# cloneofsimo/paint-with-words-sd

Hardware: NVIDIA H100
Metric: unet_steps_per_sec_512sq_cfg (higher is better)
Workload: dtype f16

## Files before the change

paint_with_words_sd_b200/csrc/attn_tc.cuh:

```cuda
#pragma once
#include "mma_sm90.cuh"
#include "pww_common.cuh"
#include "xattn_core.cuh"

namespace pww {
namespace fa {

constexpr int kThreads = core::kThreads;
constexpr int kBM = core::kBM;
constexpr int kBN = 64;

template <int D>
struct Cfg {
  using T_ = core::Tile<D>;
  static constexpr uint32_t KVBYTES = kBN * T_::LD * 2;
  static constexpr uint32_t OFF_KV = T_::QBYTES;
  static constexpr uint32_t SMEM = T_::QBYTES + 2 * 2 * KVBYTES;
  static_assert(SMEM <= 232448, "shared memory budget");
};

template <typename E>
struct Params {
  const E* q;
  const E* k;
  const E* v;
  E* out;
  int B, H, N;
  int64_t bs, rs;
  int64_t o_bs, o_rs;
  float scale;
};

template <int D, typename E>
constexpr int kMinBlocks = (D == 80 && std::is_same_v<E, __nv_bfloat16>) ? 1 : 0;

template <int D, typename E>
__global__ void __launch_bounds__(kThreads, kMinBlocks<D, E>) attn_fwd_kernel(const Params<E> p) {
  using C = core::Tile<D>;
  using CF = Cfg<D>;
  extern __shared__ __align__(128) unsigned char smem[];
  const uint32_t smem0 = ptx::smem_u32(smem);
  const int warp = threadIdx.x >> 5, lane = threadIdx.x & 31;
  const int qtiles = (p.N + kBM - 1) / kBM;
  const int bh = blockIdx.x / qtiles, qt = blockIdx.x - bh * qtiles;
  const int b = bh / p.H, h = bh - b * p.H;
  const int row_base = qt * kBM;
  const E* qb = p.q + (int64_t)b * p.bs + h * D;
  const E* kb = p.k + (int64_t)b * p.bs + h * D;
  const E* vb = p.v + (int64_t)b * p.bs + h * D;
  const int ntiles = (p.N + kBN - 1) / kBN;
  auto issue_kv = [&](int j) {
    const uint32_t st = smem0 + CF::OFF_KV + (j & 1) * 2 * CF::KVBYTES;
    const int rows = p.N - j * kBN < kBN ? p.N - j * kBN : kBN;
    core::load_rows<D>(st, kb + (int64_t)j * kBN * p.rs, p.rs, kBN, rows);
    core::load_rows<D>(st + CF::KVBYTES, vb + (int64_t)j * kBN * p.rs, p.rs, kBN, rows);
    ptx::cp_async_commit();
  };
  {
    const int rows = p.N - row_base < kBM ? p.N - row_base : kBM;
    core::load_rows<D>(smem0, qb + (int64_t)row_base * p.rs, p.rs, kBM, rows);
  }
  issue_kv(0);
  uint32_t qa[C::KS][4];
  float o[C::NT][4], m0, m1, l0, l1;
  core::warp_online_begin<D>(o, m0, m1, l0, l1);
  const float sl2 = p.scale * 1.4426950408889634f;
  const uint32_t qs = smem0 + (uint32_t)(warp * 16 * C::LD) * 2u;
#pragma unroll 1
  for (int jt = 0; jt < ntiles; ++jt) {
    if (jt + 1 < ntiles) {
      issue_kv(jt + 1);
      ptx::cp_async_wait<1>();
    } else {
      ptx::cp_async_wait<0>();
    }
    __syncthreads();
    if (jt == 0) {
#pragma unroll
      for (int kk = 0; kk < C::KS; ++kk)
        ptx::ldsm_x4(qs + (uint32_t)((lane & 15) * C::LD + kk * 16 + (lane >> 4) * 8) * 2u, qa[kk][0], qa[kk][1], qa[kk][2], qa[kk][3]);
    }
    const uint32_t ks = smem0 + CF::OFF_KV + (jt & 1) * 2 * CF::KVBYTES, vs = ks + CF::KVBYTES;
    float s[kBN / 8][4];
#pragma unroll
    for (int j = 0; j < kBN / 8; ++j) s[j][0] = s[j][1] = s[j][2] = s[j][3] = 0.f;
#pragma unroll
    for (int kk = 0; kk < C::KS; ++kk) {
#pragma unroll
      for (int jp = 0; jp < kBN / 16; ++jp) {
        const int t = 16 * jp + (lane & 7) + ((lane >> 4) << 3), d = kk * 16 + ((lane >> 3) & 1) * 8;
        uint32_t b0, b1, b2, b3;
        ptx::ldsm_x4(ks + (uint32_t)(t * C::LD + d) * 2u, b0, b1, b2, b3);
        ptx::mma16816<E>(s[2 * jp], qa[kk], b0, b1);
        ptx::mma16816<E>(s[2 * jp + 1], qa[kk], b2, b3);
      }
    }
    core::warp_online_chunk<D, E>(s, p.N - jt * kBN, sl2, vs, lane, o, m0, m1, l0, l1);
    __syncthreads();
  }
  core::warp_online_end<D>(o, l0, l1);
  core::warp_store<D>(o, smem + warp * 16 * C::LD * 2, lane, p.out + (int64_t)b * p.o_bs + h * D, p.o_rs,
                      row_base + warp * 16, p.N);
}

template <int D, typename E>
cudaError_t launch(const void* q, const void* k, const void* v, void* out, int B, int H, int N, int64_t bs, int64_t rs,
                   int64_t o_bs, int64_t o_rs, float scale, cudaStream_t s) {
  using CF = Cfg<D>;
  Params<E> p;
  p.q = (const E*)q; p.k = (const E*)k; p.v = (const E*)v; p.out = (E*)out;
  p.B = B; p.H = H; p.N = N; p.bs = bs; p.rs = rs; p.o_bs = o_bs; p.o_rs = o_rs; p.scale = scale;
  const cudaError_t e = allow_dynamic_smem<attn_fwd_kernel<D, E>>(CF::SMEM);
  if (e != cudaSuccess) return e;
  const long long grid = (long long)B * H * ((N + kBM - 1) / kBM);
  if (grid > 0x7fffffffLL) return cudaErrorInvalidConfiguration;
  attn_fwd_kernel<D, E><<<(unsigned)grid, kThreads, CF::SMEM, s>>>(p);
  return cudaGetLastError();
}

}
}
```

paint_with_words_sd_b200/csrc/mma_sm90.cuh:

```cuda
#pragma once
#include <cuda_runtime.h>
#include <stdint.h>

#include <type_traits>

#include "pww_common.cuh"

namespace pww {
namespace ptx {

__device__ __forceinline__ uint32_t smem_u32(const void* p) { return (uint32_t)__cvta_generic_to_shared(p); }

__device__ __forceinline__ void cp_async16(uint32_t dst, const void* src, uint32_t src_bytes) {
  asm volatile("cp.async.cg.shared.global [%0], [%1], 16, %2;" ::"r"(dst), "l"(src), "r"(src_bytes) : "memory");
}
__device__ __forceinline__ void cp_async_commit() { asm volatile("cp.async.commit_group;" ::: "memory"); }
template <int N>
__device__ __forceinline__ void cp_async_wait() { asm volatile("cp.async.wait_group %0;" ::"n"(N) : "memory"); }

__device__ __forceinline__ void ldsm_x4(uint32_t addr, uint32_t& r0, uint32_t& r1, uint32_t& r2, uint32_t& r3) {
  asm volatile("ldmatrix.sync.aligned.m8n8.x4.shared.b16 {%0, %1, %2, %3}, [%4];"
               : "=r"(r0), "=r"(r1), "=r"(r2), "=r"(r3) : "r"(addr));
}
__device__ __forceinline__ void ldsm_x4_t(uint32_t addr, uint32_t& r0, uint32_t& r1, uint32_t& r2, uint32_t& r3) {
  asm volatile("ldmatrix.sync.aligned.m8n8.x4.trans.shared.b16 {%0, %1, %2, %3}, [%4];"
               : "=r"(r0), "=r"(r1), "=r"(r2), "=r"(r3) : "r"(addr));
}
__device__ __forceinline__ void ldsm_x2_t(uint32_t addr, uint32_t& r0, uint32_t& r1) {
  asm volatile("ldmatrix.sync.aligned.m8n8.x2.trans.shared.b16 {%0, %1}, [%2];" : "=r"(r0), "=r"(r1) : "r"(addr));
}

template <typename E>
__device__ __forceinline__ void mma16816(float* c, const uint32_t* a, uint32_t b0, uint32_t b1) {
  static_assert(std::is_same_v<E, __half> || std::is_same_v<E, __nv_bfloat16>, "fp16 or bf16 operands");
  if constexpr (std::is_same_v<E, __half>) {
    asm volatile(
        "mma.sync.aligned.m16n8k16.row.col.f32.f16.f16.f32 {%0, %1, %2, %3}, {%4, %5, %6, %7}, {%8, %9}, "
        "{%0, %1, %2, %3};"
        : "+f"(c[0]), "+f"(c[1]), "+f"(c[2]), "+f"(c[3])
        : "r"(a[0]), "r"(a[1]), "r"(a[2]), "r"(a[3]), "r"(b0), "r"(b1));
  } else {
    asm volatile(
        "mma.sync.aligned.m16n8k16.row.col.f32.bf16.bf16.f32 {%0, %1, %2, %3}, {%4, %5, %6, %7}, {%8, %9}, "
        "{%0, %1, %2, %3};"
        : "+f"(c[0]), "+f"(c[1]), "+f"(c[2]), "+f"(c[3])
        : "r"(a[0]), "r"(a[1]), "r"(a[2]), "r"(a[3]), "r"(b0), "r"(b1));
  }
}

__device__ __forceinline__ float ex2(float x) {
  float y;
  asm("ex2.approx.ftz.f32 %0, %1;" : "=f"(y) : "f"(x));
  return y;
}
template <typename E>
__device__ __forceinline__ uint32_t pack2(float lo, float hi) {
  const typename Elem<E>::E2 h = Elem<E>::from_float2(lo, hi);
  return *reinterpret_cast<const uint32_t*>(&h);
}
template <typename E>
__device__ __forceinline__ float2 unpack2(uint32_t v) {
  return Elem<E>::to_float2(*reinterpret_cast<const typename Elem<E>::E2*>(&v));
}
__device__ __forceinline__ unsigned long long ld_acquire_gpu_u64(const unsigned long long* p) {
  unsigned long long v;
  asm volatile("ld.acquire.gpu.global.u64 %0, [%1];" : "=l"(v) : "l"(p) : "memory");
  return v;
}

}
}
```

paint_with_words_sd_b200/csrc/xattn_core.cuh:

```cuda
#pragma once
#include "mma_sm90.cuh"
#include "pww_common.cuh"

namespace pww {
namespace core {

constexpr int kBM = 128;
constexpr int kTP = 80;
constexpr int kWarps = 8;
constexpr int kThreads = kWarps * 32;

template <int D>
struct Tile {
  static_assert(D == 40 || D == 64 || D == 80 || D == 160, "head dims of SD1.5 (40 / 80 / 160) and SD2.x (64)");
  static constexpr int DP = (D + 15) / 16 * 16;
  static constexpr int LD = DP + 8;
  static constexpr int KS = DP / 16;
  static constexpr int NT = D / 8;
  static constexpr uint32_t QBYTES = kBM * LD * 2;
  static constexpr uint32_t KBYTES = kTP * LD * 2;
};

template <int D, typename E>
__device__ __forceinline__ void load_rows(uint32_t dst, const E* src, int64_t rs, int nrows, int valid) {
  using C = Tile<D>;
  constexpr int CH = C::DP / 8, DCH = D / 8;
  for (int idx = threadIdx.x; idx < nrows * CH; idx += blockDim.x) {
    const int r = idx / CH, c = idx - r * CH;
    const bool ok = r < valid && c < DCH;
    ptx::cp_async16(dst + (uint32_t)(r * C::LD + c * 8) * 2u, ok ? (const void*)(src + (int64_t)r * rs + c * 8) : (const void*)src,
                    ok ? 16u : 0u);
  }
}

template <int D, typename E>
__device__ __forceinline__ void warp_qk(uint32_t qs, uint32_t ks, int lane, float (&s)[10][4]) {
  using C = Tile<D>;
#pragma unroll
  for (int j = 0; j < 10; ++j) s[j][0] = s[j][1] = s[j][2] = s[j][3] = 0.f;
#pragma unroll
  for (int kk = 0; kk < C::KS; ++kk) {
    uint32_t a[4];
    ptx::ldsm_x4(qs + (uint32_t)((lane & 15) * C::LD + kk * 16 + (lane >> 4) * 8) * 2u, a[0], a[1], a[2], a[3]);
#pragma unroll
    for (int jp = 0; jp < 5; ++jp) {
      const int t = 16 * jp + (lane & 7) + ((lane >> 4) << 3), d = kk * 16 + ((lane >> 3) & 1) * 8;
      uint32_t b0, b1, b2, b3;
      ptx::ldsm_x4(ks + (uint32_t)(t * C::LD + d) * 2u, b0, b1, b2, b3);
      ptx::mma16816<E>(s[2 * jp], a, b0, b1);
      ptx::mma16816<E>(s[2 * jp + 1], a, b2, b3);
    }
  }
}

__device__ __forceinline__ int tok(int j, int e, int lane) { return 8 * j + 2 * (lane & 3) + (e & 1); }

template <int D, typename E>
__device__ __forceinline__ void warp_store(const float (&o)[Tile<D>::NT][4], unsigned char* stage, int lane, E* out,
                                           int64_t o_rs, int row0, int N) {
  using C = Tile<D>;
  __syncwarp();
  const int g = lane >> 2, q = lane & 3;
#pragma unroll
  for (int j = 0; j < C::NT; ++j) {
    *reinterpret_cast<uint32_t*>(stage + (g * C::LD + 8 * j + 2 * q) * 2) = ptx::pack2<E>(o[j][0], o[j][1]);
    *reinterpret_cast<uint32_t*>(stage + ((g + 8) * C::LD + 8 * j + 2 * q) * 2) = ptx::pack2<E>(o[j][2], o[j][3]);
  }
  __syncwarp();
  for (int idx = lane; idx < 16 * C::NT; idx += 32) {
    const int r = idx / C::NT, c = idx - r * C::NT;
    if (row0 + r < N)
      *reinterpret_cast<uint4*>(out + (int64_t)(row0 + r) * o_rs + c * 8) =
          *reinterpret_cast<const uint4*>(stage + (r * C::LD + c * 8) * 2);
  }
  __syncwarp();
}

constexpr int kChunk = 77;
constexpr int kMaxChunks = 3;
__host__ __device__ __forceinline__ constexpr int chunks_of(int T) { return T <= kTP ? 1 : T / kChunk; }
__host__ __device__ __forceinline__ constexpr bool supported_keys(int T) {
  return T <= kTP || T == 2 * kChunk || T == kMaxChunks * kChunk;
}
template <int KC>
__host__ __device__ __forceinline__ constexpr int chunk_keys(int T) { return KC == 1 ? T : kChunk; }

template <int D, int KC, typename E>
__device__ __forceinline__ void load_operands(uint32_t st, const XattnParams<E>& p, int b, int h, int tile, bool with_v) {
  using C = Tile<D>;
  const int rows = p.N - tile * kBM;
  load_rows<D>(st, p.q + (int64_t)b * p.q_bs + (int64_t)tile * kBM * p.q_rs + h * D, p.q_rs, kBM, rows < kBM ? rows : kBM);
  const int kv = chunk_keys<KC>(p.T);
#pragma unroll 1
  for (int c = 0; c < KC; ++c) {
    const int64_t off = (int64_t)b * p.k_bs + (int64_t)c * kChunk * p.k_rs + h * D;
    load_rows<D>(st + C::QBYTES + c * C::KBYTES, p.k + off, p.k_rs, kTP, kv);
    if (with_v) load_rows<D>(st + C::QBYTES + (KC + c) * C::KBYTES, p.v + off, p.k_rs, kTP, kv);
  }
}

template <int D>
__device__ __forceinline__ void warp_online_begin(float (&o)[Tile<D>::NT][4], float& m0, float& m1, float& l0, float& l1) {
#pragma unroll
  for (int j = 0; j < Tile<D>::NT; ++j) o[j][0] = o[j][1] = o[j][2] = o[j][3] = 0.f;
  m0 = m1 = -INFINITY;
  l0 = l1 = 0.f;
}

struct NoPHook {
  template <int NK>
  __device__ __forceinline__ void operator()(const uint32_t (&)[NK][4], float, float) const {}
};

template <int D, typename E, int NJ, typename Hook = NoPHook>
__device__ __forceinline__ void warp_online_chunk(float (&s)[NJ][4], int kv, float sl2, uint32_t vs, int lane,
                                                  float (&o)[Tile<D>::NT][4], float& m0, float& m1, float& l0, float& l1,
                                                  const Hook& hook = Hook{}) {
  static_assert(NJ % 2 == 0, "P V takes two n-tiles of P per k-step");
  using C = Tile<D>;
  float t0 = -INFINITY, t1 = -INFINITY;
#pragma unroll
  for (int j = 0; j < NJ; ++j)
#pragma unroll
    for (int e = 0; e < 4; ++e) {
      if (tok(j, e, lane) >= kv) s[j][e] = -INFINITY;
      if (e < 2) t0 = fmaxf(t0, s[j][e]); else t1 = fmaxf(t1, s[j][e]);
    }
  t0 = fmaxf(t0, __shfl_xor_sync(0xffffffffu, t0, 1));
  t0 = fmaxf(t0, __shfl_xor_sync(0xffffffffu, t0, 2));
  t1 = fmaxf(t1, __shfl_xor_sync(0xffffffffu, t1, 1));
  t1 = fmaxf(t1, __shfl_xor_sync(0xffffffffu, t1, 2));
  const float mn0 = fmaxf(m0, t0), mn1 = fmaxf(m1, t1);
  const float a0 = ptx::ex2((m0 - mn0) * sl2), a1 = ptx::ex2((m1 - mn1) * sl2);
  m0 = mn0; m1 = mn1;
  const float n0 = -mn0 * sl2, n1 = -mn1 * sl2;
  uint32_t pa[NJ / 2][4];
  float r0 = 0.f, r1 = 0.f;
#pragma unroll
  for (int j = 0; j < NJ; ++j) {
    const uint32_t p01 = ptx::pack2<E>(ptx::ex2(fmaf(s[j][0], sl2, n0)), ptx::ex2(fmaf(s[j][1], sl2, n0)));
    const uint32_t p23 = ptx::pack2<E>(ptx::ex2(fmaf(s[j][2], sl2, n1)), ptx::ex2(fmaf(s[j][3], sl2, n1)));
    const float2 f01 = ptx::unpack2<E>(p01), f23 = ptx::unpack2<E>(p23);
    r0 += f01.x + f01.y;
    r1 += f23.x + f23.y;
    pa[j >> 1][(j & 1) * 2] = p01;
    pa[j >> 1][(j & 1) * 2 + 1] = p23;
  }
  l0 = l0 * a0 + r0;
  l1 = l1 * a1 + r1;
#pragma unroll
  for (int j = 0; j < C::NT; ++j) {
    o[j][0] *= a0; o[j][1] *= a0; o[j][2] *= a1; o[j][3] *= a1;
  }
#pragma unroll
  for (int kk = 0; kk < NJ / 2; ++kk) {
    const int t = 16 * kk + (lane & 7) + ((lane >> 3) & 1) * 8;
#pragma unroll
    for (int jp = 0; jp < C::NT / 2; ++jp) {
      uint32_t b0, b1, b2, b3;
      ptx::ldsm_x4_t(vs + (uint32_t)(t * C::LD + 16 * jp + (lane >> 4) * 8) * 2u, b0, b1, b2, b3);
      ptx::mma16816<E>(o[2 * jp], pa[kk], b0, b1);
      ptx::mma16816<E>(o[2 * jp + 1], pa[kk], b2, b3);
    }
    if constexpr (C::NT & 1) {
      uint32_t b0, b1;
      ptx::ldsm_x2_t(vs + (uint32_t)(t * C::LD + 8 * (C::NT - 1)) * 2u, b0, b1);
      ptx::mma16816<E>(o[C::NT - 1], pa[kk], b0, b1);
    }
  }
  hook(pa, a0, a1);
}

template <int D>
__device__ __forceinline__ void warp_online_end(float (&o)[Tile<D>::NT][4], float l0, float l1) {
  l0 += __shfl_xor_sync(0xffffffffu, l0, 1);
  l0 += __shfl_xor_sync(0xffffffffu, l0, 2);
  l1 += __shfl_xor_sync(0xffffffffu, l1, 1);
  l1 += __shfl_xor_sync(0xffffffffu, l1, 2);
  const float i0 = 1.f / l0, i1 = 1.f / l1;
#pragma unroll
  for (int j = 0; j < Tile<D>::NT; ++j) {
    o[j][0] *= i0; o[j][1] *= i0; o[j][2] *= i1; o[j][3] *= i1;
  }
}

constexpr int kRegions = 16;

template <typename E, int NK>
__device__ __forceinline__ void warp_region_chunk(const uint32_t (&pa)[NK][4], float a0, float a1, const int8_t* rt,
                                                  int lane, float (&rm)[2][4]) {
#pragma unroll
  for (int j = 0; j < 2; ++j) {
    rm[j][0] *= a0; rm[j][1] *= a0; rm[j][2] *= a1; rm[j][3] *= a1;
  }
  const int r = lane >> 2;
#pragma unroll
  for (int kk = 0; kk < NK; ++kk) {
    const int t = 16 * kk + 2 * (lane & 3);
    const int i0 = __ldg(rt + t), i1 = __ldg(rt + t + 1), i2 = __ldg(rt + t + 8), i3 = __ldg(rt + t + 9);
#pragma unroll
    for (int j = 0; j < 2; ++j) {
      const int slot = r + 8 * j;
      const uint32_t b0 = ptx::pack2<E>(i0 == slot ? 1.f : 0.f, i1 == slot ? 1.f : 0.f);
      const uint32_t b1 = ptx::pack2<E>(i2 == slot ? 1.f : 0.f, i3 == slot ? 1.f : 0.f);
      ptx::mma16816<E>(rm[j], pa[kk], b0, b1);
    }
  }
}

__device__ __forceinline__ void warp_region_add(const float (&rm)[2][4], float l0, float l1, float* acc, int row0, int N,
                                                int lane) {
  l0 += __shfl_xor_sync(0xffffffffu, l0, 1);
  l0 += __shfl_xor_sync(0xffffffffu, l0, 2);
  l1 += __shfl_xor_sync(0xffffffffu, l1, 1);
  l1 += __shfl_xor_sync(0xffffffffu, l1, 2);
  const float inv[2] = {1.f / l0, 1.f / l1};
  const int g = lane >> 2, q = lane & 3;
#pragma unroll
  for (int hf = 0; hf < 2; ++hf) {
    const int row = row0 + g + 8 * hf;
    if (row >= N) continue;
    float* a = acc + (int64_t)row * kRegions + 2 * q;
#pragma unroll
    for (int j = 0; j < 2; ++j) {
      a[8 * j] += rm[j][2 * hf] * inv[hf];
      a[8 * j + 1] += rm[j][2 * hf + 1] * inv[hf];
    }
  }
}

template <typename E>
__device__ __forceinline__ void warp_stat(const float (&s)[10][4], int T, int rows_left, int lane, bool is_max, float& vmax,
                                          float& sum, float& sumsq) {
  const int g = lane >> 2;
#pragma unroll
  for (int j = 0; j < 10; ++j)
#pragma unroll
    for (int e = 0; e < 4; ++e) {
      const bool ok = tok(j, e, lane) < T && (g + (e >> 1) * 8) < rows_left;
      if (is_max) {
        if (ok) vmax = fmaxf(vmax, s[j][e]);
      } else if (ok) {
        const float h = round_to<E>(s[j][e]);
        sum += h;
        sumsq = fmaf(h, h, sumsq);
      }
    }
}

__device__ __forceinline__ void warp_reduce_stat(double& m, double& a, double& q) {
#pragma unroll
  for (int o = 16; o > 0; o >>= 1) {
    m = fmax(m, __shfl_xor_sync(0xffffffffu, m, o));
    a += __shfl_xor_sync(0xffffffffu, a, o);
    q += __shfl_xor_sync(0xffffffffu, q, o);
  }
}

template <typename E>
__device__ __forceinline__ float stat_value(const XattnParams<E>& p, bool is_max, double m, double a, double q) {
  const double cnt = (double)p.H * (double)p.N * (double)p.T;
  double r;
  if (is_max) {
    r = m;
  } else {
    const double var = (q - a * a / cnt) / (cnt - 1.0);
    r = sqrt(var > 0.0 ? var : 0.0);
  }
  return round_to<E>((float)r);
}

}
}
```

Measured before the change: 160.0.

## Port self-attention kernel from mma.sync to Hopper wgmma with swizzled smem

Replaces the warp-level mma.sync and ldmatrix attention inner loop with warpgroup wgmma: QK^T runs from smem descriptors over 128B-swizzled tiles, and PV uses register-A wgmma. The softmax row sum is folded into the PV MMA by appending a constant-one column to V, and the unmasked tiles take a no-mask path. It also uses a larger key tile for head dim 40 and a two-stage prefetch issued after the barrier. This is meant to cut ldmatrix and issue overhead and raise tensor core throughput, at the cost of extra padding columns, fp16 rounding of the row sum, and a fragile descriptor and swizzle setup.

```diff
diff --git a/paint_with_words_sd_b200/csrc/attn_tc.cuh b/paint_with_words_sd_b200/csrc/attn_tc.cuh
--- a/paint_with_words_sd_b200/csrc/attn_tc.cuh
+++ b/paint_with_words_sd_b200/csrc/attn_tc.cuh
@@ -8,16 +8,6 @@
 
 constexpr int kThreads = core::kThreads;
 constexpr int kBM = core::kBM;
-constexpr int kBN = 64;
-
-template <int D>
-struct Cfg {
-  using T_ = core::Tile<D>;
-  static constexpr uint32_t KVBYTES = kBN * T_::LD * 2;
-  static constexpr uint32_t OFF_KV = T_::QBYTES;
-  static constexpr uint32_t SMEM = T_::QBYTES + 2 * 2 * KVBYTES;
-  static_assert(SMEM <= 232448, "shared memory budget");
-};
 
 template <typename E>
 struct Params {
@@ -31,15 +21,55 @@
   float scale;
 };
 
-template <int D, typename E>
-constexpr int kMinBlocks = (D == 80 && std::is_same_v<E, __nv_bfloat16>) ? 1 : 0;
+template <int D>
+struct WgCfg {
+  static constexpr int BN = D == 40 ? 128 : 64;
+  static constexpr int DP = core::Tile<D>::DP;
+  static constexpr int KS = DP / 16;
+  static constexpr int NO = D / 8 + 1;
+  static constexpr int KA = (DP / 8 + 7) / 8, VA = (NO + 7) / 8;
+  static constexpr uint32_t QBYTES = KA * kBM * 128, KBYTES = KA * BN * 128, VBYTES = VA * BN * 128;
+  static constexpr uint32_t STAGE = KBYTES + VBYTES;
+  static constexpr uint32_t SMEM = 1024 + QBYTES + 2 * STAGE;
+  static constexpr int MIN_BLOCKS = D <= 80 ? 2 : 1;
+  static_assert(SMEM * MIN_BLOCKS <= 227 * 1024, "shared memory budget");
+  static_assert(kBM * core::Tile<D>::LD * 2 <= QBYTES + 2 * STAGE, "the output staging fits the operand buffers");
+};
+
+template <int ROWS>
+__device__ __forceinline__ uint32_t sw128_off(int r, int c) {
+  return (uint32_t)((c >> 3) * ROWS * 128 + r * 128 + (((c & 7) ^ (r & 7)) << 4));
+}
+
+template <int ROWS, int D, typename E>
+__device__ __forceinline__ void copy_rows(uint32_t dst, const E* src, int64_t rs, int valid) {
+  constexpr int TPR = kThreads / ROWS, DC = D / 8;
+  const int r = threadIdx.x / TPR, c0 = threadIdx.x % TPR;
+  const bool ok = r < valid;
+  const E* row = src + (int64_t)r * rs;
+#pragma unroll
+  for (int i = 0; i < (DC + TPR - 1) / TPR; ++i) {
+    const int c = c0 + TPR * i;
+    if (DC % TPR == 0 || c < DC)
+      ptx::cp_async16(dst + sw128_off<ROWS>(r, c), ok ? (const void*)(row + c * 8) : (const void*)src, ok ? 16u : 0u);
+  }
+}
+
+template <int ROWS, int D>
+__device__ __forceinline__ void put_constant_chunk(unsigned char* dst, uint32_t first_word) {
+  constexpr int TPR = kThreads / ROWS;
+  if (threadIdx.x % TPR == 0)
+    *reinterpret_cast<uint4*>(dst + sw128_off<ROWS>(threadIdx.x / TPR, D / 8)) = make_uint4(first_word, 0u, 0u, 0u);
+}
 
 template <int D, typename E>
-__global__ void __launch_bounds__(kThreads, kMinBlocks<D, E>) attn_fwd_kernel(const Params<E> p) {
+__global__ void __launch_bounds__(kThreads, WgCfg<D>::MIN_BLOCKS) attn_fwd_kernel(const Params<E> p) {
   using C = core::Tile<D>;
-  using CF = Cfg<D>;
+  using W = WgCfg<D>;
+  constexpr int BN = W::BN;
   extern __shared__ __align__(128) unsigned char smem[];
-  const uint32_t smem0 = ptx::smem_u32(smem);
+  const uint32_t raw = ptx::smem_u32(smem), base = (raw + 1023u) & ~1023u;
+  unsigned char* const gbase = smem + (base - raw);
   const int warp = threadIdx.x >> 5, lane = threadIdx.x & 31;
   const int qtiles = (p.N + kBM - 1) / kBM;
   const int bh = blockIdx.x / qtiles, qt = blockIdx.x - bh * qtiles;
@@ -48,73 +78,88 @@
   const E* qb = p.q + (int64_t)b * p.bs + h * D;
   const E* kb = p.k + (int64_t)b * p.bs + h * D;
   const E* vb = p.v + (int64_t)b * p.bs + h * D;
-  const int ntiles = (p.N + kBN - 1) / kBN;
+  const int ntiles = (p.N + BN - 1) / BN;
   auto issue_kv = [&](int j) {
-    const uint32_t st = smem0 + CF::OFF_KV + (j & 1) * 2 * CF::KVBYTES;
-    const int rows = p.N - j * kBN < kBN ? p.N - j * kBN : kBN;
-    core::load_rows<D>(st, kb + (int64_t)j * kBN * p.rs, p.rs, kBN, rows);
-    core::load_rows<D>(st + CF::KVBYTES, vb + (int64_t)j * kBN * p.rs, p.rs, kBN, rows);
+    const uint32_t st = base + W::QBYTES + (j & 1) * W::STAGE;
+    const int rows = p.N - j * BN < BN ? p.N - j * BN : BN;
+    copy_rows<BN, D>(st, kb + (int64_t)j * BN * p.rs, p.rs, rows);
+    copy_rows<BN, D>(st + W::KBYTES, vb + (int64_t)j * BN * p.rs, p.rs, rows);
     ptx::cp_async_commit();
   };
   {
     const int rows = p.N - row_base < kBM ? p.N - row_base : kBM;
-    core::load_rows<D>(smem0, qb + (int64_t)row_base * p.rs, p.rs, kBM, rows);
+    copy_rows<kBM, D>(base, qb + (int64_t)row_base * p.rs, p.rs, rows);
   }
   issue_kv(0);
-  uint32_t qa[C::KS][4];
-  float o[C::NT][4], m0, m1, l0, l1;
-  core::warp_online_begin<D>(o, m0, m1, l0, l1);
+  if (ntiles > 1) issue_kv(1);
+  {
+    const uint32_t one = ptx::pack2<E>(1.f, 0.f);
+    if constexpr (W::DP > D) put_constant_chunk<kBM, D>(gbase, 0u);
+#pragma unroll
+    for (int st = 0; st < 2; ++st) {
+      unsigned char* const s = gbase + W::QBYTES + st * W::STAGE;
+      if constexpr (W::DP > D) put_constant_chunk<BN, D>(s, 0u);
+      put_constant_chunk<BN, D>(s + W::KBYTES, one);
+    }
+  }
+  float o[W::NO][4], m0 = -INFINITY, m1 = -INFINITY;
+#pragma unroll
+  for (int j = 0; j < W::NO; ++j) o[j][0] = o[j][1] = o[j][2] = o[j][3] = 0.f;
+  auto& od = reinterpret_cast<float(&)[C::NT][4]>(o);
+  float l0 = 0.f, l1 = 0.f;
   const float sl2 = p.scale * 1.4426950408889634f;
-  const uint32_t qs = smem0 + (uint32_t)(warp * 16 * C::LD) * 2u;
+  const uint32_t qs = base + (uint32_t)(warp >> 2) * 64 * 128;
 #pragma unroll 1
   for (int jt = 0; jt < ntiles; ++jt) {
-    if (jt + 1 < ntiles) {
-      issue_kv(jt + 1);
-      ptx::cp_async_wait<1>();
-    } else {
-      ptx::cp_async_wait<0>();
-    }
+    if (jt + 1 < ntiles) ptx::cp_async_wait<1>(); else ptx::cp_async_wait<0>();
+    ptx::fence_proxy_async();
     __syncthreads();
-    if (jt == 0) {
+    const uint32_t ks = base + W::QBYTES + (jt & 1) * W::STAGE, vs = ks + W::KBYTES;
+    float s[BN / 8][4];
+    ptx::wgmma_fence();
 #pragma unroll
-      for (int kk = 0; kk < C::KS; ++kk)
-        ptx::ldsm_x4(qs + (uint32_t)((lane & 15) * C::LD + kk * 16 + (lane >> 4) * 8) * 2u, qa[kk][0], qa[kk][1], qa[kk][2], qa[kk][3]);
-    }
-    const uint32_t ks = smem0 + CF::OFF_KV + (jt & 1) * 2 * CF::KVBYTES, vs = ks + CF::KVBYTES;
-    float s[kBN / 8][4];
+    for (int kk = 0; kk < W::KS; ++kk)
+      ptx::wgmma_ss<BN, E>(s, ptx::sw128_desc(qs + (kk >> 2) * kBM * 128 + (kk & 3) * 32, 16, 1024),
+                           ptx::sw128_desc(ks + (kk >> 2) * BN * 128 + (kk & 3) * 32, 16, 1024), kk > 0);
+    ptx::wgmma_commit();
+    ptx::wgmma_wait<0>();
+    ptx::reg_fence(s);
+    uint32_t pa[BN / 16][4];
+    float a0, a1;
+    const int kv = p.N - jt * BN;
+    if (kv >= BN)
+      core::warp_online_softmax<D, E, BN / 8, false, false>(s, kv, sl2, lane, od, m0, m1, l0, l1, pa, a0, a1);
+    else
+      core::warp_online_softmax<D, E, BN / 8, true, false>(s, kv, sl2, lane, od, m0, m1, l0, l1, pa, a0, a1);
+    o[W::NO - 1][0] *= a0; o[W::NO - 1][1] *= a0; o[W::NO - 1][2] *= a1; o[W::NO - 1][3] *= a1;
+    ptx::reg_fence(o);
+    ptx::wgmma_fence();
 #pragma unroll
-    for (int j = 0; j < kBN / 8; ++j) s[j][0] = s[j][1] = s[j][2] = s[j][3] = 0.f;
-#pragma unroll
-    for (int kk = 0; kk < C::KS; ++kk) {
-#pragma unroll
-      for (int jp = 0; jp < kBN / 16; ++jp) {
-        const int t = 16 * jp + (lane & 7) + ((lane >> 4) << 3), d = kk * 16 + ((lane >> 3) & 1) * 8;
-        uint32_t b0, b1, b2, b3;
-        ptx::ldsm_x4(ks + (uint32_t)(t * C::LD + d) * 2u, b0, b1, b2, b3);
-        ptx::mma16816<E>(s[2 * jp], qa[kk], b0, b1);
-        ptx::mma16816<E>(s[2 * jp + 1], qa[kk], b2, b3);
-      }
-    }
-    core::warp_online_chunk<D, E>(s, p.N - jt * kBN, sl2, vs, lane, o, m0, m1, l0, l1);
+    for (int kk = 0; kk < BN / 16; ++kk)
+      ptx::wgmma_rs<8 * W::NO, E>(o, pa[kk], ptx::sw128_desc(vs + kk * 16 * 128, BN * 128, 1024));
+    ptx::wgmma_commit();
+    ptx::wgmma_wait<0>();
+    ptx::reg_fence(o);
     __syncthreads();
+    if (jt + 2 < ntiles) issue_kv(jt + 2);
   }
-  core::warp_online_end<D>(o, l0, l1);
-  core::warp_store<D>(o, smem + warp * 16 * C::LD * 2, lane, p.out + (int64_t)b * p.o_bs + h * D, p.o_rs,
+  core::warp_online_end<D>(od, o[W::NO - 1][0] + o[W::NO - 1][1], o[W::NO - 1][2] + o[W::NO - 1][3]);
+  core::warp_store<D>(od, gbase + warp * 16 * C::LD * 2, lane, p.out + (int64_t)b * p.o_bs + h * D, p.o_rs,
                       row_base + warp * 16, p.N);
 }
 
 template <int D, typename E>
 cudaError_t launch(const void* q, const void* k, const void* v, void* out, int B, int H, int N, int64_t bs, int64_t rs,
                    int64_t o_bs, int64_t o_rs, float scale, cudaStream_t s) {
-  using CF = Cfg<D>;
+  using W = WgCfg<D>;
   Params<E> p;
   p.q = (const E*)q; p.k = (const E*)k; p.v = (const E*)v; p.out = (E*)out;
   p.B = B; p.H = H; p.N = N; p.bs = bs; p.rs = rs; p.o_bs = o_bs; p.o_rs = o_rs; p.scale = scale;
-  const cudaError_t e = allow_dynamic_smem<attn_fwd_kernel<D, E>>(CF::SMEM);
+  const cudaError_t e = allow_dynamic_smem<attn_fwd_kernel<D, E>>(W::SMEM);
   if (e != cudaSuccess) return e;
   const long long grid = (long long)B * H * ((N + kBM - 1) / kBM);
   if (grid > 0x7fffffffLL) return cudaErrorInvalidConfiguration;
-  attn_fwd_kernel<D, E><<<(unsigned)grid, kThreads, CF::SMEM, s>>>(p);
+  attn_fwd_kernel<D, E><<<(unsigned)grid, kThreads, W::SMEM, s>>>(p);
   return cudaGetLastError();
 }
 
diff --git a/paint_with_words_sd_b200/csrc/mma_sm90.cuh b/paint_with_words_sd_b200/csrc/mma_sm90.cuh
--- a/paint_with_words_sd_b200/csrc/mma_sm90.cuh
+++ b/paint_with_words_sd_b200/csrc/mma_sm90.cuh
@@ -48,6 +48,144 @@
   }
 }
 
+__device__ __forceinline__ uint64_t sw128_desc(uint32_t addr, uint32_t lbo, uint32_t sbo) {
+  return (uint64_t)((addr & 0x3FFFFu) >> 4) | ((uint64_t)((lbo >> 4) & 0x3FFFu) << 16) |
+         ((uint64_t)((sbo >> 4) & 0x3FFFu) << 32) | (1ull << 62);
+}
+__device__ __forceinline__ void fence_proxy_async() { asm volatile("fence.proxy.async.shared::cta;" ::: "memory"); }
+__device__ __forceinline__ void wgmma_fence() { asm volatile("wgmma.fence.sync.aligned;" ::: "memory"); }
+__device__ __forceinline__ void wgmma_commit() { asm volatile("wgmma.commit_group.sync.aligned;" ::: "memory"); }
+template <int N>
+__device__ __forceinline__ void wgmma_wait() { asm volatile("wgmma.wait_group.sync.aligned %0;" ::"n"(N) : "memory"); }
+template <int R>
+__device__ __forceinline__ void reg_fence(float (&x)[R][4]) {
+#pragma unroll
+  for (int i = 0; i < R; ++i) asm volatile("" : "+f"(x[i][0]), "+f"(x[i][1]), "+f"(x[i][2]), "+f"(x[i][3])::"memory");
+}
+
+#define PWW_WG_REGS_48 "{%0, %1, %2, %3, %4, %5, %6, %7, %8, %9, %10, %11, %12, %13, %14, %15" \
+  ", %16, %17, %18, %19, %20, %21, %22, %23}"
+#define PWW_WG_OUT_48(d) "+f"(d[0][0]), "+f"(d[0][1]), "+f"(d[0][2]), "+f"(d[0][3]), "+f"(d[1][0]), "+f"(d[1][1]), \
+  "+f"(d[1][2]), "+f"(d[1][3]), "+f"(d[2][0]), "+f"(d[2][1]), "+f"(d[2][2]), "+f"(d[2][3]), "+f"(d[3][0]), \
+  "+f"(d[3][1]), "+f"(d[3][2]), "+f"(d[3][3]), "+f"(d[4][0]), "+f"(d[4][1]), "+f"(d[4][2]), "+f"(d[4][3]), \
+  "+f"(d[5][0]), "+f"(d[5][1]), "+f"(d[5][2]), "+f"(d[5][3])
+#define PWW_WG_REGS_64 "{%0, %1, %2, %3, %4, %5, %6, %7, %8, %9, %10, %11, %12, %13, %14, %15" \
+  ", %16, %17, %18, %19, %20, %21, %22, %23, %24, %25, %26, %27, %28, %29, %30, %31}"
+#define PWW_WG_OUT_64(d) "+f"(d[0][0]), "+f"(d[0][1]), "+f"(d[0][2]), "+f"(d[0][3]), "+f"(d[1][0]), "+f"(d[1][1]), \
+  "+f"(d[1][2]), "+f"(d[1][3]), "+f"(d[2][0]), "+f"(d[2][1]), "+f"(d[2][2]), "+f"(d[2][3]), "+f"(d[3][0]), \
+  "+f"(d[3][1]), "+f"(d[3][2]), "+f"(d[3][3]), "+f"(d[4][0]), "+f"(d[4][1]), "+f"(d[4][2]), "+f"(d[4][3]), \
+  "+f"(d[5][0]), "+f"(d[5][1]), "+f"(d[5][2]), "+f"(d[5][3]), "+f"(d[6][0]), "+f"(d[6][1]), "+f"(d[6][2]), \
+  "+f"(d[6][3]), "+f"(d[7][0]), "+f"(d[7][1]), "+f"(d[7][2]), "+f"(d[7][3])
+#define PWW_WG_REGS_72 "{%0, %1, %2, %3, %4, %5, %6, %7, %8, %9, %10, %11, %12, %13, %14, %15" \
+  ", %16, %17, %18, %19, %20, %21, %22, %23, %24, %25, %26, %27, %28, %29, %30, %31" \
+  ", %32, %33, %34, %35}"
+#define PWW_WG_OUT_72(d) "+f"(d[0][0]), "+f"(d[0][1]), "+f"(d[0][2]), "+f"(d[0][3]), "+f"(d[1][0]), "+f"(d[1][1]), \
+  "+f"(d[1][2]), "+f"(d[1][3]), "+f"(d[2][0]), "+f"(d[2][1]), "+f"(d[2][2]), "+f"(d[2][3]), "+f"(d[3][0]), \
+  "+f"(d[3][1]), "+f"(d[3][2]), "+f"(d[3][3]), "+f"(d[4][0]), "+f"(d[4][1]), "+f"(d[4][2]), "+f"(d[4][3]), \
+  "+f"(d[5][0]), "+f"(d[5][1]), "+f"(d[5][2]), "+f"(d[5][3]), "+f"(d[6][0]), "+f"(d[6][1]), "+f"(d[6][2]), \
+  "+f"(d[6][3]), "+f"(d[7][0]), "+f"(d[7][1]), "+f"(d[7][2]), "+f"(d[7][3]), "+f"(d[8][0]), "+f"(d[8][1]), \
+  "+f"(d[8][2]), "+f"(d[8][3])
+#define PWW_WG_REGS_88 "{%0, %1, %2, %3, %4, %5, %6, %7, %8, %9, %10, %11, %12, %13, %14, %15" \
+  ", %16, %17, %18, %19, %20, %21, %22, %23, %24, %25, %26, %27, %28, %29, %30, %31" \
+  ", %32, %33, %34, %35, %36, %37, %38, %39, %40, %41, %42, %43}"
+#define PWW_WG_OUT_88(d) "+f"(d[0][0]), "+f"(d[0][1]), "+f"(d[0][2]), "+f"(d[0][3]), "+f"(d[1][0]), "+f"(d[1][1]), \
+  "+f"(d[1][2]), "+f"(d[1][3]), "+f"(d[2][0]), "+f"(d[2][1]), "+f"(d[2][2]), "+f"(d[2][3]), "+f"(d[3][0]), \
+  "+f"(d[3][1]), "+f"(d[3][2]), "+f"(d[3][3]), "+f"(d[4][0]), "+f"(d[4][1]), "+f"(d[4][2]), "+f"(d[4][3]), \
+  "+f"(d[5][0]), "+f"(d[5][1]), "+f"(d[5][2]), "+f"(d[5][3]), "+f"(d[6][0]), "+f"(d[6][1]), "+f"(d[6][2]), \
+  "+f"(d[6][3]), "+f"(d[7][0]), "+f"(d[7][1]), "+f"(d[7][2]), "+f"(d[7][3]), "+f"(d[8][0]), "+f"(d[8][1]), \
+  "+f"(d[8][2]), "+f"(d[8][3]), "+f"(d[9][0]), "+f"(d[9][1]), "+f"(d[9][2]), "+f"(d[9][3]), "+f"(d[10][0]), \
+  "+f"(d[10][1]), "+f"(d[10][2]), "+f"(d[10][3])
+#define PWW_WG_REGS_128 "{%0, %1, %2, %3, %4, %5, %6, %7, %8, %9, %10, %11, %12, %13, %14, %15" \
+  ", %16, %17, %18, %19, %20, %21, %22, %23, %24, %25, %26, %27, %28, %29, %30, %31" \
+  ", %32, %33, %34, %35, %36, %37, %38, %39, %40, %41, %42, %43, %44, %45, %46, %47" \
+  ", %48, %49, %50, %51, %52, %53, %54, %55, %56, %57, %58, %59, %60, %61, %62, %63}"
+#define PWW_WG_OUT_128(d) "+f"(d[0][0]), "+f"(d[0][1]), "+f"(d[0][2]), "+f"(d[0][3]), "+f"(d[1][0]), "+f"(d[1][1]), \
+  "+f"(d[1][2]), "+f"(d[1][3]), "+f"(d[2][0]), "+f"(d[2][1]), "+f"(d[2][2]), "+f"(d[2][3]), "+f"(d[3][0]), \
+  "+f"(d[3][1]), "+f"(d[3][2]), "+f"(d[3][3]), "+f"(d[4][0]), "+f"(d[4][1]), "+f"(d[4][2]), "+f"(d[4][3]), \
+  "+f"(d[5][0]), "+f"(d[5][1]), "+f"(d[5][2]), "+f"(d[5][3]), "+f"(d[6][0]), "+f"(d[6][1]), "+f"(d[6][2]), \
+  "+f"(d[6][3]), "+f"(d[7][0]), "+f"(d[7][1]), "+f"(d[7][2]), "+f"(d[7][3]), "+f"(d[8][0]), "+f"(d[8][1]), \
+  "+f"(d[8][2]), "+f"(d[8][3]), "+f"(d[9][0]), "+f"(d[9][1]), "+f"(d[9][2]), "+f"(d[9][3]), "+f"(d[10][0]), \
+  "+f"(d[10][1]), "+f"(d[10][2]), "+f"(d[10][3]), "+f"(d[11][0]), "+f"(d[11][1]), "+f"(d[11][2]), "+f"(d[11][3]), \
+  "+f"(d[12][0]), "+f"(d[12][1]), "+f"(d[12][2]), "+f"(d[12][3]), "+f"(d[13][0]), "+f"(d[13][1]), "+f"(d[13][2]), \
+  "+f"(d[13][3]), "+f"(d[14][0]), "+f"(d[14][1]), "+f"(d[14][2]), "+f"(d[14][3]), "+f"(d[15][0]), "+f"(d[15][1]), \
+  "+f"(d[15][2]), "+f"(d[15][3])
+#define PWW_WG_REGS_168 "{%0, %1, %2, %3, %4, %5, %6, %7, %8, %9, %10, %11, %12, %13, %14, %15" \
+  ", %16, %17, %18, %19, %20, %21, %22, %23, %24, %25, %26, %27, %28, %29, %30, %31" \
+  ", %32, %33, %34, %35, %36, %37, %38, %39, %40, %41, %42, %43, %44, %45, %46, %47" \
+  ", %48, %49, %50, %51, %52, %53, %54, %55, %56, %57, %58, %59, %60, %61, %62, %63" \
+  ", %64, %65, %66, %67, %68, %69, %70, %71, %72, %73, %74, %75, %76, %77, %78, %79" \
+  ", %80, %81, %82, %83}"
+#define PWW_WG_OUT_168(d) "+f"(d[0][0]), "+f"(d[0][1]), "+f"(d[0][2]), "+f"(d[0][3]), "+f"(d[1][0]), "+f"(d[1][1]), \
+  "+f"(d[1][2]), "+f"(d[1][3]), "+f"(d[2][0]), "+f"(d[2][1]), "+f"(d[2][2]), "+f"(d[2][3]), "+f"(d[3][0]), \
+  "+f"(d[3][1]), "+f"(d[3][2]), "+f"(d[3][3]), "+f"(d[4][0]), "+f"(d[4][1]), "+f"(d[4][2]), "+f"(d[4][3]), \
+  "+f"(d[5][0]), "+f"(d[5][1]), "+f"(d[5][2]), "+f"(d[5][3]), "+f"(d[6][0]), "+f"(d[6][1]), "+f"(d[6][2]), \
+  "+f"(d[6][3]), "+f"(d[7][0]), "+f"(d[7][1]), "+f"(d[7][2]), "+f"(d[7][3]), "+f"(d[8][0]), "+f"(d[8][1]), \
+  "+f"(d[8][2]), "+f"(d[8][3]), "+f"(d[9][0]), "+f"(d[9][1]), "+f"(d[9][2]), "+f"(d[9][3]), "+f"(d[10][0]), \
+  "+f"(d[10][1]), "+f"(d[10][2]), "+f"(d[10][3]), "+f"(d[11][0]), "+f"(d[11][1]), "+f"(d[11][2]), "+f"(d[11][3]), \
+  "+f"(d[12][0]), "+f"(d[12][1]), "+f"(d[12][2]), "+f"(d[12][3]), "+f"(d[13][0]), "+f"(d[13][1]), "+f"(d[13][2]), \
+  "+f"(d[13][3]), "+f"(d[14][0]), "+f"(d[14][1]), "+f"(d[14][2]), "+f"(d[14][3]), "+f"(d[15][0]), "+f"(d[15][1]), \
+  "+f"(d[15][2]), "+f"(d[15][3]), "+f"(d[16][0]), "+f"(d[16][1]), "+f"(d[16][2]), "+f"(d[16][3]), "+f"(d[17][0]), \
+  "+f"(d[17][1]), "+f"(d[17][2]), "+f"(d[17][3]), "+f"(d[18][0]), "+f"(d[18][1]), "+f"(d[18][2]), "+f"(d[18][3]), \
+  "+f"(d[19][0]), "+f"(d[19][1]), "+f"(d[19][2]), "+f"(d[19][3]), "+f"(d[20][0]), "+f"(d[20][1]), "+f"(d[20][2]), \
+  "+f"(d[20][3])
+#define PWW_WGMMA_SS_64(T, d, da, db, sc) \
+  asm volatile("{\n.reg .pred p;\nsetp.ne.b32 p, %34, 0;\n" \
+               "wgmma.mma_async.sync.aligned.m64n64k16.f32." T "." T " " PWW_WG_REGS_64 \
+               ", %32, %33, p, 1, 1, 0, 0;\n}\n" \
+               : PWW_WG_OUT_64(d) : "l"(da), "l"(db), "r"(sc))
+#define PWW_WGMMA_SS_128(T, d, da, db, sc) \
+  asm volatile("{\n.reg .pred p;\nsetp.ne.b32 p, %66, 0;\n" \
+               "wgmma.mma_async.sync.aligned.m64n128k16.f32." T "." T " " PWW_WG_REGS_128 \
+               ", %64, %65, p, 1, 1, 0, 0;\n}\n" \
+               : PWW_WG_OUT_128(d) : "l"(da), "l"(db), "r"(sc))
+#define PWW_WGMMA_RS_48(T, d, a, db) \
+  asm volatile("{\n.reg .pred p;\nsetp.ne.b32 p, %29, 0;\n" \
+               "wgmma.mma_async.sync.aligned.m64n48k16.f32." T "." T " " PWW_WG_REGS_48 \
+               ", {%24, %25, %26, %27}, %28, p, 1, 1, 1;\n}\n" \
+               : PWW_WG_OUT_48(d) : "r"(a[0]), "r"(a[1]), "r"(a[2]), "r"(a[3]), "l"(db), "r"(1))
+#define PWW_WGMMA_RS_72(T, d, a, db) \
+  asm volatile("{\n.reg .pred p;\nsetp.ne.b32 p, %41, 0;\n" \
+               "wgmma.mma_async.sync.aligned.m64n72k16.f32." T "." T " " PWW_WG_REGS_72 \
+               ", {%36, %37, %38, %39}, %40, p, 1, 1, 1;\n}\n" \
+               : PWW_WG_OUT_72(d) : "r"(a[0]), "r"(a[1]), "r"(a[2]), "r"(a[3]), "l"(db), "r"(1))
+#define PWW_WGMMA_RS_88(T, d, a, db) \
+  asm volatile("{\n.reg .pred p;\nsetp.ne.b32 p, %49, 0;\n" \
+               "wgmma.mma_async.sync.aligned.m64n88k16.f32." T "." T " " PWW_WG_REGS_88 \
+               ", {%44, %45, %46, %47}, %48, p, 1, 1, 1;\n}\n" \
+               : PWW_WG_OUT_88(d) : "r"(a[0]), "r"(a[1]), "r"(a[2]), "r"(a[3]), "l"(db), "r"(1))
+#define PWW_WGMMA_RS_168(T, d, a, db) \
+  asm volatile("{\n.reg .pred p;\nsetp.ne.b32 p, %89, 0;\n" \
+               "wgmma.mma_async.sync.aligned.m64n168k16.f32." T "." T " " PWW_WG_REGS_168 \
+               ", {%84, %85, %86, %87}, %88, p, 1, 1, 1;\n}\n" \
+               : PWW_WG_OUT_168(d) : "r"(a[0]), "r"(a[1]), "r"(a[2]), "r"(a[3]), "l"(db), "r"(1))
+
+template <int N, typename E>
+__device__ __forceinline__ void wgmma_ss(float (&d)[N / 8][4], uint64_t da, uint64_t db, int scale_d) {
+  static_assert(std::is_same_v<E, __half> || std::is_same_v<E, __nv_bfloat16>, "fp16 or bf16 operands");
+  static_assert(N == 64 || N == 128, "key tile of the self-attention kernel");
+  constexpr bool f16 = std::is_same_v<E, __half>;
+  if constexpr (N == 64) {
+    if constexpr (f16) PWW_WGMMA_SS_64("f16", d, da, db, scale_d); else PWW_WGMMA_SS_64("bf16", d, da, db, scale_d);
+  } else {
+    if constexpr (f16) PWW_WGMMA_SS_128("f16", d, da, db, scale_d); else PWW_WGMMA_SS_128("bf16", d, da, db, scale_d);
+  }
+}
+template <int N, typename E>
+__device__ __forceinline__ void wgmma_rs(float (&d)[N / 8][4], const uint32_t (&a)[4], uint64_t db) {
+  static_assert(std::is_same_v<E, __half> || std::is_same_v<E, __nv_bfloat16>, "fp16 or bf16 operands");
+  static_assert(N == 48 || N == 72 || N == 88 || N == 168, "SD head dims 40 / 64 / 80 / 160, + 8");
+  constexpr bool f16 = std::is_same_v<E, __half>;
+  if constexpr (N == 48) {
+    if constexpr (f16) PWW_WGMMA_RS_48("f16", d, a, db); else PWW_WGMMA_RS_48("bf16", d, a, db);
+  } else if constexpr (N == 72) {
+    if constexpr (f16) PWW_WGMMA_RS_72("f16", d, a, db); else PWW_WGMMA_RS_72("bf16", d, a, db);
+  } else if constexpr (N == 88) {
+    if constexpr (f16) PWW_WGMMA_RS_88("f16", d, a, db); else PWW_WGMMA_RS_88("bf16", d, a, db);
+  } else {
+    if constexpr (f16) PWW_WGMMA_RS_168("f16", d, a, db); else PWW_WGMMA_RS_168("bf16", d, a, db);
+  }
+}
+
 __device__ __forceinline__ float ex2(float x) {
   float y;
   asm("ex2.approx.ftz.f32 %0, %1;" : "=f"(y) : "f"(x));
diff --git a/paint_with_words_sd_b200/csrc/xattn_core.cuh b/paint_with_words_sd_b200/csrc/xattn_core.cuh
--- a/paint_with_words_sd_b200/csrc/xattn_core.cuh
+++ b/paint_with_words_sd_b200/csrc/xattn_core.cuh
@@ -112,10 +112,10 @@
   __device__ __forceinline__ void operator()(const uint32_t (&)[NK][4], float, float) const {}
 };
 
-template <int D, typename E, int NJ, typename Hook = NoPHook>
-__device__ __forceinline__ void warp_online_chunk(float (&s)[NJ][4], int kv, float sl2, uint32_t vs, int lane,
-                                                  float (&o)[Tile<D>::NT][4], float& m0, float& m1, float& l0, float& l1,
-                                                  const Hook& hook = Hook{}) {
+template <int D, typename E, int NJ, bool MASK = true, bool SUM = true>
+__device__ __forceinline__ void warp_online_softmax(float (&s)[NJ][4], int kv, float sl2, int lane,
+                                                    float (&o)[Tile<D>::NT][4], float& m0, float& m1, float& l0,
+                                                    float& l1, uint32_t (&pa)[NJ / 2][4], float& a0, float& a1) {
   static_assert(NJ % 2 == 0, "P V takes two n-tiles of P per k-step");
   using C = Tile<D>;
   float t0 = -INFINITY, t1 = -INFINITY;
@@ -123,7 +123,7 @@
   for (int j = 0; j < NJ; ++j)
 #pragma unroll
     for (int e = 0; e < 4; ++e) {
-      if (tok(j, e, lane) >= kv) s[j][e] = -INFINITY;
+      if (MASK && tok(j, e, lane) >= kv) s[j][e] = -INFINITY;
       if (e < 2) t0 = fmaxf(t0, s[j][e]); else t1 = fmaxf(t1, s[j][e]);
     }
   t0 = fmaxf(t0, __shfl_xor_sync(0xffffffffu, t0, 1));
@@ -131,29 +131,37 @@
   t1 = fmaxf(t1, __shfl_xor_sync(0xffffffffu, t1, 1));
   t1 = fmaxf(t1, __shfl_xor_sync(0xffffffffu, t1, 2));
   const float mn0 = fmaxf(m0, t0), mn1 = fmaxf(m1, t1);
-  const float a0 = ptx::ex2((m0 - mn0) * sl2), a1 = ptx::ex2((m1 - mn1) * sl2);
+  a0 = ptx::ex2((m0 - mn0) * sl2); a1 = ptx::ex2((m1 - mn1) * sl2);
   m0 = mn0; m1 = mn1;
   const float n0 = -mn0 * sl2, n1 = -mn1 * sl2;
-  uint32_t pa[NJ / 2][4];
   float r0 = 0.f, r1 = 0.f;
 #pragma unroll
   for (int j = 0; j < NJ; ++j) {
     const uint32_t p01 = ptx::pack2<E>(ptx::ex2(fmaf(s[j][0], sl2, n0)), ptx::ex2(fmaf(s[j][1], sl2, n0)));
     const uint32_t p23 = ptx::pack2<E>(ptx::ex2(fmaf(s[j][2], sl2, n1)), ptx::ex2(fmaf(s[j][3], sl2, n1)));
-    const float2 f01 = ptx::unpack2<E>(p01), f23 = ptx::unpack2<E>(p23);
-    r0 += f01.x + f01.y;
-    r1 += f23.x + f23.y;
+    if constexpr (SUM) {
+      const float2 f01 = ptx::unpack2<E>(p01), f23 = ptx::unpack2<E>(p23);
+      r0 += f01.x + f01.y;
+      r1 += f23.x + f23.y;
+    }
     pa[j >> 1][(j & 1) * 2] = p01;
     pa[j >> 1][(j & 1) * 2 + 1] = p23;
   }
-  l0 = l0 * a0 + r0;
-  l1 = l1 * a1 + r1;
+  if constexpr (SUM) {
+    l0 = l0 * a0 + r0;
+    l1 = l1 * a1 + r1;
+  }
 #pragma unroll
   for (int j = 0; j < C::NT; ++j) {
     o[j][0] *= a0; o[j][1] *= a0; o[j][2] *= a1; o[j][3] *= a1;
   }
-#pragma unroll
-  for (int kk = 0; kk < NJ / 2; ++kk) {
+}
+
+template <int D, typename E, int NK>
+__device__ __forceinline__ void warp_pv(const uint32_t (&pa)[NK][4], uint32_t vs, int lane, float (&o)[Tile<D>::NT][4]) {
+  using C = Tile<D>;
+#pragma unroll
+  for (int kk = 0; kk < NK; ++kk) {
     const int t = 16 * kk + (lane & 7) + ((lane >> 3) & 1) * 8;
 #pragma unroll
     for (int jp = 0; jp < C::NT / 2; ++jp) {
@@ -168,6 +176,16 @@
       ptx::mma16816<E>(o[C::NT - 1], pa[kk], b0, b1);
     }
   }
+}
+
+template <int D, typename E, int NJ, typename Hook = NoPHook>
+__device__ __forceinline__ void warp_online_chunk(float (&s)[NJ][4], int kv, float sl2, uint32_t vs, int lane,
+                                                  float (&o)[Tile<D>::NT][4], float& m0, float& m1, float& l0, float& l1,
+                                                  const Hook& hook = Hook{}) {
+  uint32_t pa[NJ / 2][4];
+  float a0, a1;
+  warp_online_softmax<D, E, NJ>(s, kv, sl2, lane, o, m0, m1, l0, l1, pa, a0, a1);
+  warp_pv<D, E, NJ / 2>(pa, vs, lane, o);
   hook(pa, a0, a1);
 }
 
```

After: 161.9, median of 6. 1.2% higher.
